# SysCV/LiDAR_snow_sim

Hardware: NVIDIA H100
Metric: augmented LiDAR points/sec (higher is better)
Workload: dtype f64

## Files before the change

### lidar_snow_sim_b200/csrc/prepass.cu

```cuda
#include "common.cuh"

namespace {

constexpr int PP_TPB = 256;
constexpr int HIST_NX = 50, HIST_NY = 2555;
constexpr int RANSAC_T = 128;


struct PreArgs {
    const float *pts;
    const int64_t *cloud_off;
    const int32_t *cloud_cnt;
    int raise_few;
    int range_min_ground;
    int range64;
    int n_clouds;
    double delta;
    double noise_floor;
    int flat_earth;
    int have_plane;
    CloudPre *cp;
    float *win;
    float *stage;
    int *tile_cnt;
    const int32_t *tile_base;
    double *rec_norm;
    unsigned char *rec_bin;
    int *rec_cnt;
    double *trial;
    double *partial;
    int max_blocks;
    int *status;
    const int32_t *ymins_in;
    int32_t *ymins;
};

__device__ __forceinline__ float range32(float x, float y, float z)
{
    return __fsqrt_rn(__fadd_rn(__fadd_rn(__fmul_rn(x, x), __fmul_rn(y, y)), __fmul_rn(z, z)));
}

__device__ __forceinline__ unsigned long long splitmix64(unsigned long long x)
{
    x += 0x9E3779B97F4A7C15ULL;
    x = (x ^ (x >> 30)) * 0xBF58476D1CE4E5B9ULL;
    x = (x ^ (x >> 27)) * 0x94D049BB133111EBULL;
    return x ^ (x >> 31);
}

template <int NV>
__device__ void block_sum(double (&v)[NV], double *smem )
{
    const int lane = threadIdx.x & 31, warp = threadIdx.x >> 5, nw = blockDim.x >> 5;
#pragma unroll
    for (int k = 0; k < NV; k++)
#pragma unroll
        for (int s = 16; s > 0; s >>= 1) v[k] += __shfl_down_sync(0xffffffffu, v[k], s);
    __syncthreads();
    if (lane == 0)
#pragma unroll
        for (int k = 0; k < NV; k++) smem[k * nw + warp] = v[k];
    __syncthreads();
    if (threadIdx.x == 0)
#pragma unroll
        for (int k = 0; k < NV; k++) {
            double s = 0.0;
            for (int q = 0; q < nw; q++) s += smem[k * nw + q];
            v[k] = s;
        }
}

constexpr int WTILE = 256;

__device__ __forceinline__ bool lss_in_window(float x, float y, float z)
{
    const float lim = __fsub_rn(-1.86f, __fmul_rn(0.01f, x));
    return (z < -1.55f) && (z > lim) && (x > 10.0f) && (x < 70.0f) && (y > -3.0f) && (y < 3.0f);
}
__device__ __forceinline__ int64_t lss_window_tile0(int64_t cloud_begin, int b) { return cloud_begin / 32 + b; }

__global__ void __launch_bounds__(WTILE) k_window_tiles(PreArgs a)
{
    const int b = blockIdx.y;
    const int64_t beg = a.cloud_off[b];
    const int n = (a.cloud_cnt ? a.cloud_cnt[b] : (int)(a.cloud_off[b + 1] - beg));
    const int w0 = blockIdx.x * WTILE + (threadIdx.x & ~31);
    if (w0 >= n) return;
    const int lane = threadIdx.x & 31;
    const int i = w0 + lane;
    float x = 0, y = 0, z = 0;
    bool in = false;
    if (i < n) {
        const float *r = a.pts + (beg + i) * 5;
        x = __ldcs(r); y = __ldcs(r + 1); z = __ldcs(r + 2);
        in = lss_in_window(x, y, z);
    }
    const unsigned m = __ballot_sync(0xffffffffu, in);
    if (in) {
        float *o = a.stage + (beg + w0 + __popc(m & ((1u << lane) - 1u))) * 3;
        o[0] = x; o[1] = y; o[2] = z;
    }
    if (lane == 0) a.tile_cnt[lss_window_tile0(beg, b) + w0 / 32] = __popc(m);
}

__device__ __forceinline__ unsigned f2key(float f)
{
    unsigned u = __float_as_uint(f);
    return (u & 0x80000000u) ? ~u : (u | 0x80000000u);
}
__device__ __forceinline__ float key2f(unsigned k)
{
    unsigned u = (k & 0x80000000u) ? (k & 0x7fffffffu) : ~k;
    return __uint_as_float(u);
}

__device__ float block_select(const float *win, int K, int kth, int mode, float centre, unsigned *hist ,
                              unsigned *bcast )
{
    unsigned prefix = 0, mask = 0;
    int k = kth;
    for (int shift = 24; shift >= 0; shift -= 8) {
        for (int q = threadIdx.x; q < 256; q += blockDim.x) hist[q] = 0;
        __syncthreads();
        for (int i = threadIdx.x; i < K; i += blockDim.x) {
            float v = win[3 * (size_t)i + 2];
            if (mode) v = fabsf(__fsub_rn(v, centre));
            const unsigned key = f2key(v);
            if ((key & mask) == prefix) atomicAdd(&hist[(key >> shift) & 255u], 1u);
        }
        __syncthreads();
        if (threadIdx.x == 0) {
            int acc = 0;
            unsigned d = 0;
            for (; d < 256; d++) {
                if (acc + (int)hist[d] > k) break;
                acc += (int)hist[d];
            }
            bcast[0] = d;
            bcast[1] = (unsigned)(k - acc);
        }
        __syncthreads();
        prefix |= bcast[0] << shift;
        mask |= 255u << shift;
        k = (int)bcast[1];
        __syncthreads();
    }
    return key2f(prefix);
}

__device__ float block_median(const float *win, int K, int mode, float centre, unsigned *hist, unsigned *bcast)
{
    const float hi = block_select(win, K, K / 2, mode, centre, hist, bcast);
    if (K & 1) return hi;
    const float lo = block_select(win, K, K / 2 - 1, mode, centre, hist, bcast);
    return __fmul_rn(__fadd_rn(lo, hi), 0.5f);
}

__global__ void __launch_bounds__(1024) k_window_gather_mad(PreArgs a)
{
    extern __shared__ int prefix[];
    __shared__ int wsum[32];
    __shared__ int run_s;
    __shared__ unsigned hist[256];
    __shared__ unsigned bcast[2];
    const int b = blockIdx.x;
    const int64_t beg = a.cloud_off[b];
    const int n = (a.cloud_cnt ? a.cloud_cnt[b] : (int)(a.cloud_off[b + 1] - beg));
    const int n_tiles = (n + 31) / 32;
    const int *cnt = a.tile_cnt + lss_window_tile0(beg, b);
    const int tid = threadIdx.x, lane = tid & 31, warp = tid >> 5;
    if (tid == 0) run_s = 0;
    __syncthreads();
    for (int base = 0; base < n_tiles; base += 1024) {
        const int t = base + tid;
        const int v = t < n_tiles ? cnt[t] : 0;
        int incl = v;
#pragma unroll
        for (int s = 1; s < 32; s <<= 1) { const int o = __shfl_up_sync(0xffffffffu, incl, s); if (lane >= s) incl += o; }
        if (lane == 31) wsum[warp] = incl;
        __syncthreads();
        int o = run_s;
        for (int wv = 0; wv < warp; wv++) o += wsum[wv];
        if (t < n_tiles) prefix[t] = o + incl - v;
        __syncthreads();
        if (tid == 1023) run_s = o + incl;
        __syncthreads();
    }
    if (tid == 0) { prefix[n_tiles] = run_s; a.cp[b].n_window = run_s; }
    __syncthreads();
    const int K = prefix[n_tiles];
    float *win = a.win + beg * 3;
    for (int o = tid; o < K; o += blockDim.x) {
        int lo = 0, hi = n_tiles;
        while (hi - lo > 1) { const int mid = (lo + hi) >> 1; if (prefix[mid] <= o) lo = mid; else hi = mid; }
        const float *src = a.stage + (beg + (int64_t)lo * 32 + (o - prefix[lo])) * 3;
        float *dst = win + (int64_t)o * 3;
        dst[0] = src[0]; dst[1] = src[1]; dst[2] = src[2];
    }
    if (K <= 5) return;
    __syncthreads();
    const float med = block_median(win, K, 0, 0.0f, hist, bcast);
    const float mad = block_median(win, K, 1, med, hist, bcast);
    if (threadIdx.x == 0) { a.cp[b].z_med = med; a.cp[b].mad = mad; }
}

__global__ void __launch_bounds__(PP_TPB) k_ransac_trials(PreArgs a)
{
    __shared__ double red[5 * (PP_TPB / 32)];
    __shared__ double model[4];
    const int b = blockIdx.y, t = blockIdx.x;
    const int K = a.cp[b].n_window;
    double *out = a.trial + ((size_t)b * RANSAC_T + t) * 8;
    if (K <= 5) { if (threadIdx.x == 0) out[5] = 0.0; return; }
    const float *win = a.win + a.cloud_off[b] * 3;
    if (threadIdx.x == 0) {
        unsigned long long s = splitmix64(0x5851F42D4C957F2DULL ^ ((unsigned long long)(unsigned)K << 32) ^ (unsigned)t);
        int i0 = (int)(s % (unsigned)K);
        s = splitmix64(s);
        int i1 = (int)(s % (unsigned)(K - 1));
        if (i1 >= i0) i1++;
        s = splitmix64(s);
        int i2 = (int)(s % (unsigned)(K - 2));
        const int lo = i0 < i1 ? i0 : i1, hi = i0 < i1 ? i1 : i0;
        if (i2 >= lo) i2++;
        if (i2 >= hi) i2++;
        const double x0 = win[3 * i0], y0 = win[3 * i0 + 1], z0 = win[3 * i0 + 2];
        const double x1 = win[3 * i1] - x0, y1 = win[3 * i1 + 1] - y0, z1 = win[3 * i1 + 2] - z0;
        const double x2 = win[3 * i2] - x0, y2 = win[3 * i2 + 1] - y0, z2 = win[3 * i2 + 2] - z0;
        const double det = x1 * y2 - x2 * y1;
        double valid = 0.0, pa = 0, pb = 0, pc = 0;
        if (fabs(det) > 1e-9) {
            pa = (z1 * y2 - z2 * y1) / det;
            pb = (x1 * z2 - x2 * z1) / det;
            pc = z0 - pa * x0 - pb * y0;
            valid = 1.0;
        }
        model[0] = pa; model[1] = pb; model[2] = pc; model[3] = valid;
    }
    __syncthreads();
    if (model[3] == 0.0) { if (threadIdx.x == 0) out[5] = 0.0; return; }
    const double pa = model[0], pb = model[1], pc = model[2];
    const double thr = (double)a.cp[b].mad;
    double v[5] = {0, 0, 0, 0, 0};
    for (int i = threadIdx.x; i < K; i += PP_TPB) {
        const double x = win[3 * i], y = win[3 * i + 1], z = win[3 * i + 2];
        const double r = z - (pa * x + pb * y + pc);
        const double r2 = r * r;
        if (r2 <= thr) { v[0] += 1.0; v[1] += r2; v[2] += z; v[3] += z * z; }
    }
    block_sum<5>(v, red);
    if (threadIdx.x == 0) {
        const double n = v[0];
        const double ss_tot = v[3] - (n > 0 ? v[2] * v[2] / n : 0.0);
        out[0] = n;
        out[1] = (n > 0 && ss_tot > 0) ? 1.0 - v[1] / ss_tot : -1e300;
        out[2] = pa; out[3] = pb; out[4] = pc;
        out[5] = n >= 3 ? 1.0 : 0.0;
    }
}

__global__ void __launch_bounds__(PP_TPB) k_ransac_refit(PreArgs a)
{
    __shared__ double red[6 * (PP_TPB / 32)];
    __shared__ double bc[8];
    const int b = blockIdx.x;
    CloudPre &cp = a.cp[b];
    const int K = cp.n_window;
    if (threadIdx.x < 32) {
        int best = -1;
        double bn = -1, bs = -1e301;
        for (int t = threadIdx.x; t < RANSAC_T && K > 5; t += 32) {
            const double *tr = a.trial + ((size_t)b * RANSAC_T + t) * 8;
            if (tr[5] == 0.0) continue;
            if (tr[0] > bn || (tr[0] == bn && tr[1] > bs)) { bn = tr[0]; bs = tr[1]; best = t; }
        }
#pragma unroll
        for (int sft = 16; sft > 0; sft >>= 1) {
            const double on = __shfl_xor_sync(0xffffffffu, bn, sft), os = __shfl_xor_sync(0xffffffffu, bs, sft);
            const int ob = __shfl_xor_sync(0xffffffffu, best, sft);
            const bool take = ob >= 0 && (best < 0 || on > bn || (on == bn && (os > bs || (os == bs && ob < best))));
            if (take) { bn = on; bs = os; best = ob; }
        }
        if (threadIdx.x == 0) {
        cp.best_trial = best;
        bc[0] = (double)best;
        if (best >= 0) {
            const double *tr = a.trial + ((size_t)b * RANSAC_T + best) * 8;
            bc[1] = tr[2]; bc[2] = tr[3]; bc[3] = tr[4];
        }
        }
    }
    __syncthreads();
    const int best = (int)bc[0];
    if (best < 0) {
        if (threadIdx.x == 0) { cp.w[0] = 0; cp.w[1] = 0; cp.w[2] = 1; cp.h = -1.55; cp.nw = 1.0; cp.flat = 1; }
        return;
    }
    const float *win = a.win + a.cloud_off[b] * 3;
    const double pa = bc[1], pb = bc[2], pc = bc[3], thr = (double)cp.mad;
    double m[6] = {0, 0, 0, 0, 0, 0};
    for (int i = threadIdx.x; i < K; i += PP_TPB) {
        const double x = win[3 * i], y = win[3 * i + 1], z = win[3 * i + 2];
        const double r = z - (pa * x + pb * y + pc);
        if (r * r <= thr) { m[0] += 1.0; m[1] += x; m[2] += y; m[3] += z; }
    }
    block_sum<6>(m, red);
    if (threadIdx.x == 0) { bc[4] = m[0]; bc[5] = m[1] / m[0]; bc[6] = m[2] / m[0]; bc[7] = m[3] / m[0]; }
    __syncthreads();
    const double xm = bc[5], ym = bc[6], zm = bc[7];
    double c[6] = {0, 0, 0, 0, 0, 0};
    for (int i = threadIdx.x; i < K; i += PP_TPB) {
        const double x = win[3 * i], y = win[3 * i + 1], z = win[3 * i + 2];
        const double r = z - (pa * x + pb * y + pc);
        if (r * r <= thr) {
            const double dx = x - xm, dy = y - ym, dz = z - zm;
            c[0] += dx * dx; c[1] += dx * dy; c[2] += dy * dy; c[3] += dx * dz; c[4] += dy * dz;
        }
    }
    block_sum<6>(c, red);
    if (threadIdx.x == 0) {
        const double det = c[0] * c[2] - c[1] * c[1];
        double fa = pa, fb = pb, fc = pc;
        if (fabs(det) > 1e-12 * (c[0] * c[2] + 1e-300)) {
            fa = (c[3] * c[2] - c[4] * c[1]) / det;
            fb = (c[0] * c[4] - c[1] * c[3]) / det;
            fc = zm - fa * xm - fb * ym;
        }
        const double nrm = sqrt(fa * fa + fb * fb + 1.0);
        cp.w[0] = fa / nrm; cp.w[1] = fb / nrm; cp.w[2] = -1.0 / nrm; cp.h = fc;
        cp.nw = sqrt(cp.w[0] * cp.w[0] + cp.w[1] * cp.w[1] + cp.w[2] * cp.w[2]);
        cp.flat = 0;
    }
}

__global__ void k_set_plane(PreArgs a, const double *plane )
{
    const int b = blockIdx.x * blockDim.x + threadIdx.x;
    if (b >= a.n_clouds) return;
    CloudPre &cp = a.cp[b];
    cp.w[0] = plane[4 * b]; cp.w[1] = plane[4 * b + 1]; cp.w[2] = plane[4 * b + 2]; cp.h = plane[4 * b + 3];
    cp.nw = sqrt(cp.w[0] * cp.w[0] + cp.w[1] * cp.w[1] + cp.w[2] * cp.w[2]);
    cp.flat = 0;
    cp.best_trial = -2;
}

struct GroundPt { bool ground; double d, cosang, norm_i; };

__device__ __forceinline__ GroundPt ground_point(const PreArgs &a, const CloudPre &cp, const float *r)
{
    GroundPt g;
    const double x = r[0], y = r[1], z = r[2];
    const double pw = lss_plane_dot(x, y, z, cp.w);
    const double hgt = pw + cp.h;
    g.ground = (hgt < a.delta) && (hgt > -a.delta);
    if (!g.ground) { g.d = 0.0; g.cosang = 0.0; g.norm_i = 0.0; return g; }
    g.d = a.range64 ? sqrt((x * x + y * y) + z * z) : (double)range32(r[0], r[1], r[2]);
    double c;
    if (a.flat_earth) c = -(z) / (g.d * 1.0);
    else c = pw / (g.d * cp.nw);
    g.cosang = (c >= -1.0 && c <= 1.0) ? c : __longlong_as_double(0x7ff8000000000000LL);
    g.norm_i = (double)r[3] / g.cosang;
    return g;
}

__device__ __forceinline__ int edge_bin(double v, double lo, double hi, int nb)
{
    if (!(v >= lo) || !(v <= hi)) return -1;
    const double step = (hi - lo) / nb;
    int k = (int)((v - lo) / step);
    k = k < 0 ? 0 : (k > nb ? nb : k);
    while (k > 0 && v < ((k == nb) ? hi : (k * step + lo))) k--;
    while (k < nb && v >= ((k + 1 == nb) ? hi : ((k + 1) * step + lo))) k++;
    if (k >= nb) k = nb - 1;
    return k;
}

__device__ __forceinline__ void intensity_edges(double ymax, double &lo, double &hi)
{
    lo = ymax == 5.0 ? 4.5 : 5.0;
    hi = ymax == 5.0 ? 5.5 : ymax;
}

__device__ __forceinline__ double nan_max(double a, double b) { return (a != a || a > b) ? a : b; }

__device__ __forceinline__ int ground_blocks(int n, int launched)
{
    return min(launched, max(1, (n + PP_TPB * 8 - 1) / (PP_TPB * 8)));
}

__global__ void __launch_bounds__(PP_TPB) k_ground_stats(PreArgs a)
{
    __shared__ double red[15 * (PP_TPB / 32)];
    __shared__ double mx[PP_TPB / 32];
    const int b = blockIdx.y;
    const CloudPre cp = a.cp[b];
    const int64_t beg = a.cloud_off[b];
    const int n = (a.cloud_cnt ? a.cloud_cnt[b] : (int)(a.cloud_off[b + 1] - beg));
    const int nb = ground_blocks(n, gridDim.x);
    if ((int)blockIdx.x >= nb) return;
    const int lane = threadIdx.x & 31;
    double v[15] = {0, 0, 0, 0, 0, 0, 0, 0, 0, 0, 0, 0, 0, 0, 0};
    double vmax = -1e300;
    for (int w0 = blockIdx.x * PP_TPB + (threadIdx.x & ~31); w0 < n; w0 += nb * PP_TPB) {
        const int i = w0 + lane;
        GroundPt g;
        g.ground = false;
        if (i < n) {
            const float *r = a.pts + (beg + i) * 5;
            const float row[4] = {__ldcs(r), __ldcs(r + 1), __ldcs(r + 2), __ldcs(r + 3)};
            g = ground_point(a, cp, row);
        }
        int bx = -1;
        if (g.ground) {
            const double dd = g.d - 30.0, yy = g.norm_i - 50.0;
            v[0] += 1.0; v[1] += dd; v[2] += yy; v[3] += dd * dd; v[4] += dd * yy;
            vmax = nan_max(vmax, g.norm_i);
            const double t = (g.d - 40.0) / 30.0, t2 = t * t;
            const double c = g.cosang, dc = g.d * g.cosang;
            v[5] += t; v[6] += t2; v[7] += t2 * t; v[8] += t2 * t2;
            v[9] += c; v[10] += c * t; v[11] += c * t2;
            v[12] += dc; v[13] += dc * t; v[14] += dc * t2;
            if (g.norm_i >= 4.5) bx = edge_bin(g.d, 10.0, 70.0, HIST_NX);
        }
        const unsigned m = __ballot_sync(0xffffffffu, bx >= 0);
        if (m) {
            int k0 = 0;
            if (lane == 0) k0 = atomicAdd(&a.rec_cnt[b], __popc(m));
            k0 = __shfl_sync(0xffffffffu, k0, 0);
            if (bx >= 0) {
                const int64_t k = beg + k0 + __popc(m & ((1u << lane) - 1u));
                a.rec_norm[k] = g.norm_i;
                a.rec_bin[k] = (unsigned char)bx;
            }
        }
    }
#pragma unroll
    for (int s = 16; s > 0; s >>= 1) vmax = nan_max(vmax, __shfl_down_sync(0xffffffffu, vmax, s));
    if ((threadIdx.x & 31) == 0) mx[threadIdx.x >> 5] = vmax;
    block_sum<15>(v, red);
    if (threadIdx.x == 0) {
        for (int q = 0; q < PP_TPB / 32; q++) vmax = nan_max(vmax, mx[q]);
        double *p = a.partial + ((size_t)b * a.max_blocks + blockIdx.x) * 16;
        for (int k = 0; k < 15; k++) p[k] = v[k];
        p[15] = vmax;
    }
}

template <int NV>
__device__ __forceinline__ void warp_reduce_partials(const double *partial, int n_blocks, double (&v)[NV], double *vmax)
{
    const int lane = threadIdx.x & 31;
#pragma unroll
    for (int k = 0; k < NV; k++) v[k] = 0.0;
    double m = -1e300;
    for (int q = lane; q < n_blocks; q += 32) {
        const double *p = partial + (size_t)q * 16;
#pragma unroll
        for (int k = 0; k < NV; k++) v[k] += p[k];
        if (vmax) m = nan_max(m, p[NV]);
    }
#pragma unroll
    for (int s = 16; s > 0; s >>= 1) {
#pragma unroll
        for (int k = 0; k < NV; k++) v[k] += __shfl_xor_sync(0xffffffffu, v[k], s);
        m = nan_max(m, __shfl_xor_sync(0xffffffffu, m, s));
    }
    if (vmax) *vmax = m;
}

#ifndef LSS_HIST_SLAB
#define LSS_HIST_SLAB 5
#endif
constexpr int HIST_SLAB = LSS_HIST_SLAB, HIST_SLABS = (HIST_NX + HIST_SLAB - 1) / HIST_SLAB, HIST_TPB = 512;

__global__ void __launch_bounds__(HIST_TPB) k_ground_hist(PreArgs a, int n_blocks)
{
    extern __shared__ unsigned hist[];
    __shared__ double stat[2];
    const int b = blockIdx.y, bx0 = blockIdx.x * HIST_SLAB;
    const int nbx = min(HIST_SLAB, HIST_NX - bx0);
    const int lane = threadIdx.x & 31, warp = threadIdx.x >> 5;
    if (warp == 0) {
        double v[15], vmax;
        const int n = a.cloud_cnt ? a.cloud_cnt[b] : (int)(a.cloud_off[b + 1] - a.cloud_off[b]);
        warp_reduce_partials<15>(a.partial + (size_t)b * a.max_blocks * 16, ground_blocks(n, n_blocks), v, &vmax);
        if (lane == 0) {
            stat[0] = v[0];
            stat[1] = fabs(vmax);
            if (blockIdx.x == 0) {
                CloudPre &cp = a.cp[b];
                cp.n_ground = (int)v[0];
                cp.mom[0] = v[0];
                for (int k = 0; k < 10; k++) cp.mom[1 + k] = v[5 + k];
                cp.ymax = fabs(vmax);
                if (v[0] >= 3.0) {
                    const double n = v[0], mx_ = v[1] / n, my_ = v[2] / n;
                    const double sxx = v[3] - n * mx_ * mx_, sxy = v[4] - n * mx_ * my_;
                    const double slope = sxy / sxx;
                    cp.lin[0] = slope;
                    cp.lin[1] = (my_ + 50.0) - slope * (mx_ + 30.0);
                } else {
                    cp.lin[0] = cp.lin[1] = 0.0;
                    if (a.raise_few) atomicMax(a.status, LSS_ERR_TOO_FEW_GROUND);
                }
                if (v[0] >= (double)a.range_min_ground && !lss_intensity_range_ok(cp.ymax))
                    atomicMax(a.status, LSS_ERR_INTENSITY_RANGE);
            }
        }
    }
    __syncthreads();
    const int n_ground = (int)stat[0];
    const double ymax = stat[1];
    if (n_ground < 3 || !lss_intensity_range_ok(ymax)) return;
    double ylo, yhi;
    intensity_edges(ymax, ylo, yhi);
    int32_t *ymins = a.ymins + b * HIST_NX + bx0;
    if (a.ymins_in) {
        for (int k = threadIdx.x; k < nbx; k += HIST_TPB) {
            const int inj = a.ymins_in[b * HIST_NX + bx0 + k];
            ymins[k] = inj < 0 ? 0 : (inj >= HIST_NY ? HIST_NY - 1 : inj);
        }
        return;
    }
    for (int k = threadIdx.x; k < nbx * HIST_NY; k += HIST_TPB) hist[k] = 0;
    __syncthreads();
    const int64_t beg = a.cloud_off[b];
    const int n_rec = a.rec_cnt[b];
    const unsigned char *bins = a.rec_bin + beg;
    const double *norms = a.rec_norm + beg;
    constexpr int U = 4;
    for (int k0 = threadIdx.x; k0 < n_rec; k0 += U * HIST_TPB) {
        int rel[U];
#pragma unroll
        for (int u = 0; u < U; u++) {
            const int k = k0 + u * HIST_TPB;
            rel[u] = k < n_rec ? (int)bins[k] - bx0 : -1;
        }
#pragma unroll
        for (int u = 0; u < U; u++)
            if ((unsigned)rel[u] < (unsigned)nbx) {
                const int by = edge_bin(norms[k0 + u * HIST_TPB], ylo, yhi, HIST_NY);
                if (by >= 0) atomicAdd(&hist[rel[u] * HIST_NY + by], 1u);
            }
    }
    __syncthreads();
    for (int w = warp; w < nbx; w += HIST_TPB / 32) {
        unsigned best = 0xffffffffu;
        int bidx = 0x7fffffff;
        for (int k = lane; k < HIST_NY; k += 32) {
            unsigned c = hist[w * HIST_NY + k];
            if (c == 0) c = (unsigned)n_ground;
            if (c < best) { best = c; bidx = k; }
        }
        for (int s = 16; s > 0; s >>= 1) {
            const unsigned ob = __shfl_down_sync(0xffffffffu, best, s);
            const int oi = __shfl_down_sync(0xffffffffu, bidx, s);
            if (ob < best || (ob == best && oi < bidx)) { best = ob; bidx = oi; }
        }
        if (lane == 0) ymins[w] = bidx;
    }
}

__device__ __forceinline__ bool minima_point(int k, int bidx, double ylo, double yhi, double ystep, double &x, double &y)
{
    y = (bidx == HIST_NY) ? yhi : __dadd_rn(__dmul_rn((double)bidx, ystep), ylo);
    const double e0 = k * (60.0 / HIST_NX) + 10.0;
    const double e1 = (k + 1 == HIST_NX) ? 70.0 : ((k + 1) * (60.0 / HIST_NX) + 10.0);
    x = (e0 + e1) / 2;
    return y > 5.0;
}

__global__ void k_poly_solve(PreArgs a, double *poly_out , double *plane_out ,
                             double *fit_out , int32_t *ymins_out )
{
    const int b = blockIdx.x;
    CloudPre &cp = a.cp[b];
    if (threadIdx.x != 0) return;
    const bool picked = cp.n_ground >= 3 && lss_intensity_range_ok(cp.ymax);
    if (cp.n_ground >= 3) {
        const int32_t *ymins = a.ymins + b * HIST_NX;
        double ylo, yhi;
        intensity_edges(cp.ymax, ylo, yhi);
        const double ystep = (yhi - ylo) / HIST_NY;
        int m = 0;
        double sx = 0, sy = 0, x, y;
        for (int k = 0; k < HIST_NX && picked; k++)
            if (minima_point(k, ymins[k], ylo, yhi, ystep, x, y)) { m++; sx += x; sy += y; }
        if (m > 3) {
            const double mx_ = sx / m, my_ = sy / m;
            double sxx = 0, sxy = 0;
            for (int k = 0; k < HIST_NX; k++)
                if (minima_point(k, ymins[k], ylo, yhi, ystep, x, y)) { sxx += (x - mx_) * (x - mx_); sxy += (x - mx_) * (y - my_); }
            cp.pmin[0] = sxy / sxx;
            cp.pmin[1] = my_ - cp.pmin[0] * mx_;
        } else {
            cp.pmin[0] = cp.lin[0];
            cp.pmin[1] = cp.lin[1];
        }
    }
    double s[8];
    s[0] = cp.mom[0]; s[1] = cp.mom[1]; s[2] = cp.mom[2]; s[3] = cp.mom[3]; s[4] = cp.mom[4];
    for (int k = 0; k < 3; k++) s[5 + k] = a.noise_floor * (cp.pmin[0] * cp.mom[8 + k] + cp.pmin[1] * cp.mom[5 + k]);
    double A[3][4] = {{s[0], s[1], s[2], s[5]}, {s[1], s[2], s[3], s[6]}, {s[2], s[3], s[4], s[7]}};
    bool ok = cp.n_ground >= 3;
    for (int c = 0; c < 3 && ok; c++) {
        int piv = c;
        for (int r = c + 1; r < 3; r++) if (fabs(A[r][c]) > fabs(A[piv][c])) piv = r;
        if (fabs(A[piv][c]) < 1e-300) { ok = false; break; }
        for (int k = 0; k < 4; k++) { double t = A[c][k]; A[c][k] = A[piv][k]; A[piv][k] = t; }
        for (int r = c + 1; r < 3; r++) {
            const double f = A[r][c] / A[c][c];
            for (int k = c; k < 4; k++) A[r][k] -= f * A[c][k];
        }
    }
    double c2 = 0, c1 = 0, c0 = 0;
    if (ok) {
        c2 = A[2][3] / A[2][2];
        c1 = (A[1][3] - A[1][2] * c2) / A[1][1];
        c0 = (A[0][3] - A[0][1] * c1 - A[0][2] * c2) / A[0][0];
    }
    const double m = 40.0, sc = 30.0;
    cp.poly[0] = c2 / (sc * sc);
    cp.poly[1] = c1 / sc - 2.0 * c2 * m / (sc * sc);
    cp.poly[2] = c0 - c1 * m / sc + c2 * m * m / (sc * sc);
    if (poly_out) { poly_out[3 * b] = cp.poly[0]; poly_out[3 * b + 1] = cp.poly[1]; poly_out[3 * b + 2] = cp.poly[2]; }
    if (plane_out) { plane_out[4 * b] = cp.w[0]; plane_out[4 * b + 1] = cp.w[1]; plane_out[4 * b + 2] = cp.w[2]; plane_out[4 * b + 3] = cp.h; }
    if (fit_out) {
        double *f = fit_out + 8 * b;
        f[0] = cp.lin[0]; f[1] = cp.lin[1]; f[2] = cp.pmin[0]; f[3] = cp.pmin[1]; f[4] = cp.ymax;
        f[5] = (double)cp.n_ground; f[6] = (double)cp.n_window; f[7] = (double)cp.flat;
    }
    if (ymins_out) for (int k = 0; k < HIST_NX; k++) ymins_out[b * HIST_NX + k] = picked ? a.ymins[b * HIST_NX + k] : -1;
}

}

struct PrepassLayout { int64_t cp, rec_cnt, win, stage, tile_cnt, tile_base, trial, partial, plane_in, ymins, ymins_in, total; int max_blocks; };

static PrepassLayout prepass_layout(int64_t n_total, int n_clouds)
{
    PrepassLayout L;
    L.max_blocks = 64;
    int64_t o = 0;
    L.cp = o;       o = align_up(o + (int64_t)sizeof(CloudPre) * n_clouds, 256);
    L.rec_cnt = o;  o = align_up(o + (int64_t)n_clouds * 4, 256);
    L.win = o;      o = align_up(o + n_total * 3 * 4, 256);
    L.stage = o;    o = align_up(o + n_total * 3 * 4, 256);
    L.tile_cnt = o; o = align_up(o + (n_total / 32 + n_clouds + 2) * 4, 256);
    L.tile_base = o; o = align_up(o + (int64_t)(n_clouds + 1) * 4, 256);
    L.trial = o;    o = align_up(o + (int64_t)n_clouds * RANSAC_T * 8 * 8, 256);
    L.partial = o;  o = align_up(o + (int64_t)n_clouds * L.max_blocks * 16 * 8, 256);
    L.plane_in = o; o = align_up(o + (int64_t)n_clouds * 4 * 8, 256);
    L.ymins = o;    o = align_up(o + (int64_t)n_clouds * HIST_NX * 4, 256);
    L.ymins_in = o; o = align_up(o + (int64_t)n_clouds * HIST_NX * 4, 256);
    L.total = o;
    return L;
}

int64_t lss_prepass_ws_bytes(int64_t n_total, int n_clouds) { return prepass_layout(n_total, n_clouds).total; }

static size_t gather_dyn_smem(int64_t max_n) { return sizeof(int) * ((size_t)(max_n + 31) / 32 + 2); }

static int64_t largest_cloud(const int64_t *h_cloud_off, int n_clouds)
{
    int64_t max_n = 0;
    for (int b = 0; b < n_clouds; b++) max_n = std::max<int64_t>(max_n, h_cloud_off[b + 1] - h_cloud_off[b]);
    return max_n;
}

static lss_status gather_smem_limits(lss_engine *e, size_t &static_bytes, size_t &optin_bytes)
{
    cudaFuncAttributes fa;
    int optin = 0;
    LSS_CUDA_CHECK(e, cudaFuncGetAttributes(&fa, k_window_gather_mad));
    LSS_CUDA_CHECK(e, cudaDeviceGetAttribute(&optin, cudaDevAttrMaxSharedMemoryPerBlockOptin, e->device));
    static_bytes = fa.sharedSizeBytes;
    optin_bytes = (size_t)optin;
    return LSS_OK;
}

lss_status lss_prepass_check(lss_engine *e, const int64_t *h_cloud_off, int n_clouds, bool plane_given)
{
    if (plane_given || n_clouds <= 0) return LSS_OK;
    const int64_t max_n = largest_cloud(h_cloud_off, n_clouds);
    size_t static_bytes = 0, optin_bytes = 0;
    if (lss_status rc = gather_smem_limits(e, static_bytes, optin_bytes)) return rc;
    if (static_bytes + gather_dyn_smem(max_n) <= optin_bytes) return LSS_OK;
    const int64_t limit = ((int64_t)((optin_bytes - static_bytes) / sizeof(int)) - 2) * 32;
    char msg[256];
    snprintf(msg, sizeof(msg), "pre-pass: a cloud of %lld rows is larger than the %lld rows whose mounting window this "
             "device can gather (shared memory); give its plane or split it", (long long)max_n, (long long)limit);
    e->last_error = msg;
    return LSS_ERR_INVALID_ARG;
}

lss_status lss_prepass_run(lss_engine *e, const float *d_pts, const int64_t *d_cloud_off, const int32_t *d_cloud_cnt,
                           const int64_t *h_cloud_off, int n_clouds, double delta, double noise_floor, int flat_earth,
                           int range64, int raise_few_ground, const PrepassIO &io, void *d_ws, int64_t ws_bytes,
                           void **cloudpre_out, cudaStream_t stream)
{
    const double *h_plane_in = io.h_plane_in;
    double *d_poly_out = io.d_poly_out, *d_plane_out = io.d_plane_out;
    const int B = n_clouds;
    const int64_t N = h_cloud_off[B];
    const PrepassLayout L = prepass_layout(N, B);
    if (lss_status rc = lss_prepass_check(e, h_cloud_off, B, h_plane_in != nullptr)) return rc;
    if (ws_bytes < L.total) return lss_fail(e, LSS_ERR_WORKSPACE, "pre-pass workspace too small");
    char *ws = (char *)d_ws;
    PreArgs a;
    a.pts = d_pts;
    a.cloud_off = d_cloud_off;
    a.cloud_cnt = d_cloud_cnt;
    a.range64 = range64;
    a.raise_few = raise_few_ground;
    a.range_min_ground = io.range_min_ground;
    a.n_clouds = B;
    a.delta = delta;
    a.noise_floor = noise_floor;
    a.flat_earth = flat_earth;
    a.have_plane = h_plane_in != nullptr;
    a.cp = (CloudPre *)(ws + L.cp);
    a.win = (float *)(ws + L.win);
    a.stage = (float *)(ws + L.stage);
    a.tile_cnt = (int *)(ws + L.tile_cnt);
    a.tile_base = (const int32_t *)(ws + L.tile_base);
    a.rec_norm = (double *)(ws + L.stage);
    a.rec_bin = (unsigned char *)(ws + L.stage + N * 8);
    a.rec_cnt = (int *)(ws + L.rec_cnt);
    a.trial = (double *)(ws + L.trial);
    a.partial = (double *)(ws + L.partial);
    a.max_blocks = L.max_blocks;
    a.status = e->d_status;
    a.ymins = (int32_t *)(ws + L.ymins);
    a.ymins_in = nullptr;
    if (io.h_ymins_in) {
        LSS_CUDA_CHECK(e, lss_stage_upload(e, ws + L.ymins_in, io.h_ymins_in, sizeof(int32_t) * HIST_NX * B, stream));
        a.ymins_in = (const int32_t *)(ws + L.ymins_in);
    }
    if (cloudpre_out) *cloudpre_out = a.cp;
    const int64_t max_n = largest_cloud(h_cloud_off, B);
    int nblk = (int)std::min<int64_t>(L.max_blocks, std::max<int64_t>(1, (max_n + PP_TPB * 8 - 1) / (PP_TPB * 8)));

    {
        ZeroRegions z;
        z.add(a.cp, (size_t)(L.rec_cnt - L.cp) + sizeof(int) * B);
        LSS_CUDA_CHECK(e, lss_zero_async(e, z, stream));
    }
    {
        KernelTimer kt(e, LSS_K_PREPASS, stream);
        if (h_plane_in) {
            double *d_plane = (double *)(ws + L.plane_in);
            LSS_CUDA_CHECK(e, lss_stage_upload(e, d_plane, h_plane_in, sizeof(double) * 4 * B, stream));
            LSS_CUDA_CHECK(e, lss_launch(e, k_set_plane, (B + 127) / 128, 128, 0, stream, a, d_plane));
        } else {
            const int max_tiles = (int)std::max<int64_t>(1, (max_n + WTILE - 1) / WTILE);
            LSS_CUDA_CHECK(e, lss_launch(e, k_window_tiles, dim3(max_tiles, B), WTILE, 0, stream, a));
            const size_t gather_smem = gather_dyn_smem(max_n);
            size_t static_bytes = 0, optin_bytes = 0;
            if (lss_status rc = gather_smem_limits(e, static_bytes, optin_bytes)) return rc;
            if (static_bytes + gather_smem > 48 * 1024)
                LSS_CUDA_CHECK(e, cudaFuncSetAttribute(k_window_gather_mad, cudaFuncAttributeMaxDynamicSharedMemorySize,
                                                       (int)gather_smem));
            LSS_CUDA_CHECK(e, lss_launch(e, k_window_gather_mad, B, 1024, gather_smem, stream, a));
            LSS_CUDA_CHECK(e, lss_launch(e, k_ransac_trials, dim3(RANSAC_T, B), PP_TPB, 0, stream, a));
            LSS_CUDA_CHECK(e, lss_launch(e, k_ransac_refit, B, PP_TPB, 0, stream, a));
        }
        LSS_CUDA_CHECK(e, lss_launch(e, k_ground_stats, dim3(nblk, B), PP_TPB, 0, stream, a));
        const size_t hist_smem = sizeof(unsigned) * HIST_SLAB * HIST_NY;
        if (hist_smem > 48 * 1024)
            LSS_CUDA_CHECK(e, cudaFuncSetAttribute(k_ground_hist, cudaFuncAttributeMaxDynamicSharedMemorySize, (int)hist_smem));
        LSS_CUDA_CHECK(e, lss_launch(e, k_ground_hist, dim3(HIST_SLABS, B), HIST_TPB, hist_smem, stream, a, nblk));
        LSS_CUDA_CHECK(e, lss_launch(e, k_poly_solve, B, 32, 0, stream, a, d_poly_out, d_plane_out, io.d_fit_out,
                                     io.d_ymins_out));
    }
    return LSS_OK;
}
```

Baseline: 4.731 billion.

## Stage ground-stat point rows via cp.async into shared memory and batch record appends

The ground statistics kernel now copies up to eight segments of 5-float point rows into shared memory with cp.async, using an L2 evict-first hint, instead of strided per-thread global loads. Per-segment record counts are gathered into a block-wide prefix sum so each batch issues one atomicAdd on rec_cnt rather than one per warp. The histogram kernel loads eight records per thread and hoists the norm loads ahead of binning to raise memory-level parallelism. The staging buffer takes about 40KB of shared memory per block, which may lower occupancy. It also adds extra __syncthreads barriers.

```diff
diff --git a/lidar_snow_sim_b200/csrc/prepass.cu b/lidar_snow_sim_b200/csrc/prepass.cu
--- a/lidar_snow_sim_b200/csrc/prepass.cu
+++ b/lidar_snow_sim_b200/csrc/prepass.cu
@@ -388,49 +388,109 @@
     return min(launched, max(1, (n + PP_TPB * 8 - 1) / (PP_TPB * 8)));
 }
 
-__global__ void __launch_bounds__(PP_TPB) k_ground_stats(PreArgs a)
+__device__ __forceinline__ unsigned long long l2_evict_first()
+{
+    unsigned long long pol;
+    asm volatile("createpolicy.fractional.L2::evict_first.b64 %0, 1.0;\n" : "=l"(pol));
+    return pol;
+}
+__device__ __forceinline__ void cp_async16(void *dst, const void *src, unsigned long long pol)
+{
+    asm volatile("cp.async.cg.shared.global.L2::cache_hint [%0], [%1], 16, %2;\n"
+                 ::"r"((unsigned)__cvta_generic_to_shared(dst)), "l"(src), "l"(pol) : "memory");
+}
+__device__ __forceinline__ void cp_async4(void *dst, const void *src)
+{
+    asm volatile("cp.async.ca.shared.global [%0], [%1], 4;\n" ::"r"((unsigned)__cvta_generic_to_shared(dst)), "l"(src)
+                 : "memory");
+}
+__device__ __forceinline__ void cp_async_wait_all() { asm volatile("cp.async.wait_all;\n" ::: "memory"); }
+
+__device__ __forceinline__ void cta_copy_rows(float *dst, const float *src, int bytes, unsigned long long pol)
+{
+    char *d = (char *)dst;
+    const char *s = (const char *)src;
+    int q0 = 0;
+    if (((uintptr_t)s & 15) == 0) {
+        q0 = bytes & ~15;
+        for (int q = threadIdx.x * 16; q < q0; q += PP_TPB * 16) cp_async16(d + q, s + q, pol);
+    }
+    for (int q = q0 + threadIdx.x * 4; q < bytes; q += PP_TPB * 4) cp_async4(d + q, s + q);
+}
+
+constexpr int GS_SEGS = 8;
+
+__global__ void __launch_bounds__(PP_TPB, 3) k_ground_stats(PreArgs a)
 {
     __shared__ double red[15 * (PP_TPB / 32)];
     __shared__ double mx[PP_TPB / 32];
+    __shared__ __align__(16) float rows[GS_SEGS * PP_TPB * 5];
+    __shared__ int rec_off[GS_SEGS * (PP_TPB / 32) + 1];
     const int b = blockIdx.y;
     const CloudPre cp = a.cp[b];
     const int64_t beg = a.cloud_off[b];
     const int n = (a.cloud_cnt ? a.cloud_cnt[b] : (int)(a.cloud_off[b + 1] - beg));
     const int nb = ground_blocks(n, gridDim.x);
     if ((int)blockIdx.x >= nb) return;
-    const int lane = threadIdx.x & 31;
+    const int lane = threadIdx.x & 31, warp = threadIdx.x >> 5;
+    const unsigned long long pol = l2_evict_first();
     double v[15] = {0, 0, 0, 0, 0, 0, 0, 0, 0, 0, 0, 0, 0, 0, 0};
     double vmax = -1e300;
-    for (int w0 = blockIdx.x * PP_TPB + (threadIdx.x & ~31); w0 < n; w0 += nb * PP_TPB) {
-        const int i = w0 + lane;
-        GroundPt g;
-        g.ground = false;
-        if (i < n) {
-            const float *r = a.pts + (beg + i) * 5;
-            const float row[4] = {__ldcs(r), __ldcs(r + 1), __ldcs(r + 2), __ldcs(r + 3)};
-            g = ground_point(a, cp, row);
-        }
-        int bx = -1;
-        if (g.ground) {
-            const double dd = g.d - 30.0, yy = g.norm_i - 50.0;
-            v[0] += 1.0; v[1] += dd; v[2] += yy; v[3] += dd * dd; v[4] += dd * yy;
-            vmax = nan_max(vmax, g.norm_i);
-            const double t = (g.d - 40.0) / 30.0, t2 = t * t;
-            const double c = g.cosang, dc = g.d * g.cosang;
-            v[5] += t; v[6] += t2; v[7] += t2 * t; v[8] += t2 * t2;
-            v[9] += c; v[10] += c * t; v[11] += c * t2;
-            v[12] += dc; v[13] += dc * t; v[14] += dc * t2;
-            if (g.norm_i >= 4.5) bx = edge_bin(g.d, 10.0, 70.0, HIST_NX);
-        }
-        const unsigned m = __ballot_sync(0xffffffffu, bx >= 0);
-        if (m) {
-            int k0 = 0;
-            if (lane == 0) k0 = atomicAdd(&a.rec_cnt[b], __popc(m));
-            k0 = __shfl_sync(0xffffffffu, k0, 0);
-            if (bx >= 0) {
-                const int64_t k = beg + k0 + __popc(m & ((1u << lane) - 1u));
-                a.rec_norm[k] = g.norm_i;
-                a.rec_bin[k] = (unsigned char)bx;
+    const int r0 = (int)blockIdx.x * PP_TPB;
+    for (int j0 = 0; r0 + j0 * nb * PP_TPB < n; j0 += GS_SEGS) {
+        if (j0) __syncthreads();
+        for (int j = 0; j < GS_SEGS; j++) {
+            const int s = r0 + (j0 + j) * nb * PP_TPB;
+            if (s >= n) break;
+            cta_copy_rows(rows + j * PP_TPB * 5, a.pts + (beg + s) * 5, min(PP_TPB, n - s) * 20, pol);
+        }
+        cp_async_wait_all();
+        __syncthreads();
+        unsigned has_rec = 0;
+        for (int j = 0; j < GS_SEGS; j++) {
+            const int i = r0 + (j0 + j) * nb * PP_TPB + (int)threadIdx.x;
+            if (i >= n) break;
+            float *r = rows + (j * PP_TPB + threadIdx.x) * 5;
+            const GroundPt g = ground_point(a, cp, r);
+            if (g.ground) {
+                const double dd = g.d - 30.0, yy = g.norm_i - 50.0;
+                v[0] += 1.0; v[1] += dd; v[2] += yy; v[3] += dd * dd; v[4] += dd * yy;
+                vmax = nan_max(vmax, g.norm_i);
+                const double t = (g.d - 40.0) / 30.0, t2 = t * t;
+                const double c = g.cosang, dc = g.d * g.cosang;
+                v[5] += t; v[6] += t2; v[7] += t2 * t; v[8] += t2 * t2;
+                v[9] += c; v[10] += c * t; v[11] += c * t2;
+                v[12] += dc; v[13] += dc * t; v[14] += dc * t2;
+                const int bx = g.norm_i >= 4.5 ? edge_bin(g.d, 10.0, 70.0, HIST_NX) : -1;
+                if (bx >= 0) {
+                    const long long bits = __double_as_longlong(g.norm_i);
+                    r[0] = __int_as_float((int)bits);
+                    r[1] = __int_as_float((int)(bits >> 32));
+                    r[2] = __int_as_float(bx);
+                    has_rec |= 1u << j;
+                }
+            }
+        }
+        for (int j = 0; j < GS_SEGS; j++) {
+            const unsigned m = __ballot_sync(0xffffffffu, (has_rec >> j) & 1u);
+            if (lane == 0) rec_off[j * (PP_TPB / 32) + warp] = __popc(m);
+        }
+        __syncthreads();
+        if (threadIdx.x == 0) {
+            int acc = 0;
+            for (int q = 0; q < GS_SEGS * (PP_TPB / 32); q++) { const int c = rec_off[q]; rec_off[q] = acc; acc += c; }
+            rec_off[GS_SEGS * (PP_TPB / 32)] = acc ? atomicAdd(&a.rec_cnt[b], acc) : 0;
+        }
+        __syncthreads();
+        const int64_t base = beg + rec_off[GS_SEGS * (PP_TPB / 32)];
+        for (int j = 0; j < GS_SEGS; j++) {
+            const unsigned m = __ballot_sync(0xffffffffu, (has_rec >> j) & 1u);
+            if ((has_rec >> j) & 1u) {
+                const float *r = rows + (j * PP_TPB + threadIdx.x) * 5;
+                const int64_t k = base + rec_off[j * (PP_TPB / 32) + warp] + __popc(m & ((1u << lane) - 1u));
+                a.rec_norm[k] = __longlong_as_double((long long)(unsigned)__float_as_int(r[0]) |
+                                                     ((long long)__float_as_int(r[1]) << 32));
+                a.rec_bin[k] = (unsigned char)__float_as_int(r[2]);
             }
         }
     }
@@ -528,7 +588,7 @@
     const int n_rec = a.rec_cnt[b];
     const unsigned char *bins = a.rec_bin + beg;
     const double *norms = a.rec_norm + beg;
-    constexpr int U = 4;
+    constexpr int U = 8;
     for (int k0 = threadIdx.x; k0 < n_rec; k0 += U * HIST_TPB) {
         int rel[U];
 #pragma unroll
@@ -536,10 +596,13 @@
             const int k = k0 + u * HIST_TPB;
             rel[u] = k < n_rec ? (int)bins[k] - bx0 : -1;
         }
+        double nv[U];
+#pragma unroll
+        for (int u = 0; u < U; u++) nv[u] = (unsigned)rel[u] < (unsigned)nbx ? norms[k0 + u * HIST_TPB] : 0.0;
 #pragma unroll
         for (int u = 0; u < U; u++)
             if ((unsigned)rel[u] < (unsigned)nbx) {
-                const int by = edge_bin(norms[k0 + u * HIST_TPB], ylo, yhi, HIST_NY);
+                const int by = edge_bin(nv[u], ylo, yhi, HIST_NY);
                 if (by >= 0) atomicAdd(&hist[rel[u] * HIST_NY + by], 1u);
             }
     }
```

After: 4.779 billion (median of 6 runs). 1.0% higher.
